# SergioRAgostinho/cvxpnpl

Measured on AMD Instinct MI355X. Metric: poses/sec (batched 10x10 SDP solves/sec), higher is better.
Workload: dtype f64

## Files before the change

### cvxpnpl_amd/csrc/cvxpnpl_hip.hip

```cpp
#include <hip/hip_runtime.h>
#include <stdint.h>
#include <stdio.h>
#include <string.h>
#include <unistd.h>

#include <map>
#include <memory>
#include <mutex>
#include <vector>
#include <utility>

#include "../../include/cvxpnpl_amd.h"
#include "problem_io.h"
#include "solver_core.h"
#include "lane_core.h"
#include "batch_args.h"
#include "wave_kernel.h"
#include "quad_kernel.h"
#include "ipm_quad.h"
#include "score_kernel.h"
#include "assemble_kernel.h"
#include "synth_kernel.h"
#include "recover_kernel.h"

// ... 162 lines not shown
}

void launch_wave(int64_t wgrid, hipStream_t s, const cvxw::WaveArgs &w, const cvx::Opts &o)
{
    if (o.variant == cvx::VAR_RC) hipLaunchKernelGGL(cvxw::solve_wave_kernel<cvx::VAR_RC>, dim3((unsigned)wgrid), dim3(64 * cvxw::WPB), 0, s, w, o);
    else hipLaunchKernelGGL(cvxw::solve_wave_kernel<cvx::VAR_FULL>, dim3((unsigned)wgrid), dim3(64 * cvxw::WPB), 0, s, w, o);
}

void launch_resume(int64_t rgrid, hipStream_t s, const cvxw::WaveArgs &w, const cvx::Opts &o, int32_t *count, int32_t *entries, const double *ws, bool full)
{
    cvxw::ResumeArgs ra;
    ra.a = w; ra.o = o; ra.count_p = count; ra.entries = entries; ra.ws = ws;
    ra.ws_stride = full ? cvxw::RS_FULL : cvxw::RS_LANE; ra.ws_full = full ? 1 : 0;
    ra.count2 = nullptr; ra.entries2 = nullptr; ra.grid1 = 0;
    if (o.variant == cvx::VAR_RC) hipLaunchKernelGGL(cvxw::resume_wave_kernel_rc, dim3((unsigned)rgrid), dim3(64), 0, s, ra);
    else hipLaunchKernelGGL(cvxw::resume_wave_kernel, dim3((unsigned)rgrid), dim3(64), 0, s, ra);
}

void launch_rescue(int64_t batch, hipStream_t s, const cvxw::WaveArgs &w, const cvx::Opts &o, int32_t *count = nullptr, int32_t *entries = nullptr,
                   const double *ws = nullptr)
{
    const int64_t rgrid = batch < cvxw::RESUME_GRID_MAX ? batch : cvxw::RESUME_GRID_MAX;
    cvxw::ResumeArgs ra;
    ra.a = w; ra.o = o; ra.count_p = w.rq_count; ra.entries = w.rq_entries; ra.ws = ws; ra.ws_stride = cvxw::RS_FULL; ra.ws_full = 1;
    ra.count2 = count; ra.entries2 = entries; ra.grid1 = (int)rgrid;
    if (o.variant == cvx::VAR_RC) hipLaunchKernelGGL(cvxw::rescue_wave_kernel_rc, dim3((unsigned)(count ? 2 * rgrid : rgrid)), dim3(64), 0, s, ra);
    else hipLaunchKernelGGL(cvxw::rescue_wave_kernel, dim3((unsigned)(count ? 2 * rgrid : rgrid)), dim3(64), 0, s, ra);
}

void launch_ipm(int64_t batch, hipStream_t s, const cvxw::WaveArgs &w, const cvx::Opts &o, int32_t *count, int32_t *entries)
{
    const int64_t groups = (batch + 3) / 4;
    const int64_t grid = groups < cvxi::IPMQ_GRID_MAX ? groups : cvxi::IPMQ_GRID_MAX;
    cvxi::IpmQuadArgs ia;
    ia.batch = batch; ia.rho = o.rho; ia.rho_tail = o.rho_tail; ia.tail_from = o.tail_from;
    ia.rq_count = w.rq_count; ia.rq_entries = w.rq_entries; ia.count = count; ia.entries = entries; ia.ws = w.rq_ws; ia.stride = w.rq_stride;
    ia.entries_cap = (int)(batch + cvxw::RESUME_GRID_MAX < 0x7fffffffLL ? batch + cvxw::RESUME_GRID_MAX : 0x7fffffffLL);
    ia.qs_in = nullptr; ia.z_out = nullptr; ia.s_out = nullptr; ia.gap_out = nullptr; ia.it_out = nullptr;
    if (o.variant == cvx::VAR_RC) hipLaunchKernelGGL(cvxi::ipm_quad_kernel<cvx::VAR_RC>, dim3((unsigned)grid), dim3(64), 0, s, ia);
    else hipLaunchKernelGGL(cvxi::ipm_quad_kernel<cvx::VAR_FULL>, dim3((unsigned)grid), dim3(64), 0, s, ia);
}

int set_err(const char *what, hipError_t e)
{
    snprintf(g_err, sizeof(g_err), "%s: %s", what, hipGetErrorString(e));
    return -2;
}

cvx::Opts to_core(const cvxpnpl_opts_t *opts)
{
    cvx::Opts o = cvx::default_opts();
    if (opts) {
        o.eps = opts->eps; o.max_iters = opts->max_iters; o.rho = opts->rho; o.alpha = opts->alpha;
        o.first_check = opts->first_check; o.check_every = opts->check_every; o.res_tol = opts->res_tol;
        o.jacobi_sweeps = opts->jacobi_sweeps; o.jacobi_tol = opts->jacobi_tol; o.warm_start = opts->warm_start; o.rho_tail = opts->rho_tail; o.tail_from = opts->tail_from;
        o.variant = opts->variant;
        o.adapt_every = opts->adapt_every; o.adapt_from = opts->adapt_from; o.adapt_mu = opts->adapt_mu; o.adapt_tau = opts->adapt_tau;
        o.stall_from = opts->stall_from; o.stall_lam = opts->stall_lam; o.stall_res = opts->stall_res; o.stall_drop = opts->stall_drop;
        o.rescue_from = opts->rescue_from;
        o.f32_sweeps_until = opts->f32_sweeps_until;
        o.sweep_schedule = opts->sweep_schedule != 0;
        o.dual_shift = opts->dual_shift < 0.0 ? (opts->variant == CVXPNPL_VARIANT_RC ? 0.006 : cvx::DUAL_SHIFT_DEFAULT) : opts->dual_shift;
        o.dual_refine = opts->dual_refine != 0;
    }
    if (o.f32_sweeps_until < 0) o.f32_sweeps_until = cvx::F32_SWEEPS_DEFAULT;
    return o;
}

}

namespace cvxd {
template <int W>
__global__ void __launch_bounds__(256) calibration_copy_kernel(const char *src, char *dst, int64_t nbytes)
{
    const int64_t n = nbytes / W;
    for (int64_t i = (int64_t)blockIdx.x * 256 + threadIdx.x; i < n; i += (int64_t)gridDim.x * 256) {
        if (W == 4) reinterpret_cast<uint32_t *>(dst)[i] = reinterpret_cast<const uint32_t *>(src)[i];
        if (W == 8) reinterpret_cast<double *>(dst)[i] = reinterpret_cast<const double *>(src)[i];
        if (W == 16) reinterpret_cast<double2 *>(dst)[i] = reinterpret_cast<const double2 *>(src)[i];
    }
}
}

extern "C" {

void cvxpnpl_default_opts(cvxpnpl_opts_t *opts)
{
    cvx::Opts o = cvx::default_opts();
    opts->eps = o.eps; opts->max_iters = o.max_iters; opts->rho = o.rho; opts->alpha = o.alpha;
    opts->first_check = 0 ; opts->check_every = o.check_every; opts->res_tol = o.res_tol;
    opts->jacobi_sweeps = o.jacobi_sweeps; opts->jacobi_tol = o.jacobi_tol; opts->warm_start = o.warm_start; opts->rho_tail = o.rho_tail; opts->tail_from = o.tail_from; opts->lane_iters = -1; opts->layout = CVXPNPL_LAYOUT_AUTO; opts->variant = CVXPNPL_VARIANT_FULL;
    opts->adapt_every = o.adapt_every; opts->adapt_from = o.adapt_from; opts->adapt_mu = o.adapt_mu; opts->adapt_tau = o.adapt_tau;
    opts->stall_from = o.stall_from; opts->stall_lam = o.stall_lam; opts->stall_res = o.stall_res; opts->stall_drop = o.stall_drop;
    opts->rescue_from = o.rescue_from;
    opts->f32_sweeps_until = -1;
    opts->sweep_schedule = 1;
    opts->dual_shift = -1.0;
    opts->dual_refine = -1;
    opts->struct_size = (uint32_t)sizeof(cvxpnpl_opts_t);
}

size_t cvxpnpl_opts_size(void) { return sizeof(cvxpnpl_opts_t); }

int cvxpnpl_last_layout(void) { return g_last_layout; }

static int check_args(int64_t batch, int32_t n_p, const double *p2, const double *p3, int32_t n_l, const double *l2,
                      const double *l3, const double *K)
{
    if (batch < 0 || n_p < 0 || n_l < 0 || (n_p == 0 && n_l == 0) || !K || (n_p > 0 && (!p2 || !p3)) || (n_l > 0 && (!l2 || !l3))) {
        snprintf(g_err, sizeof(g_err), "cvxpnpl: bad arguments (batch=%lld n_p=%d n_l=%d)", (long long)batch, n_p, n_l);
        return -1;
    }
    return 0;
}

static int launch_solve(const BatchArgs &a, const cvxpnpl_opts_t *opts, void *stream)
{
    const int64_t batch = a.batch;
    if (!a.R || !a.t || !a.status) { snprintf(g_err, sizeof(g_err), "cvxpnpl: R, t and status outputs are required"); return -1; }
    if (opts && opts->struct_size != (uint32_t)sizeof(cvxpnpl_opts_t)) {
        snprintf(g_err, sizeof(g_err), "cvxpnpl: options block of %u bytes, this library's cvxpnpl_opts_t has %zu (cvxpnpl_default_opts / cvxpnpl_opts_size)",
                 opts->struct_size, sizeof(cvxpnpl_opts_t));
        return -1;
    }
    if (opts && (opts->max_iters < 1 || opts->f32_sweeps_until < -1 || opts->f32_sweeps_until > cvx::F32_SWEEPS_DEFAULT || !(opts->rho > 0) || !(opts->eps > 0) || opts->check_every < 1 || opts->first_check < 0 ||
                 (opts->variant != CVXPNPL_VARIANT_FULL && opts->variant != CVXPNPL_VARIANT_RC) || opts->adapt_every < 0 ||
                 (opts->adapt_every > 0 && !(opts->adapt_mu >= 1.0 && opts->adapt_tau > 1.0)) || opts->rescue_from < -1 || !((opts->dual_shift >= 0.0 && opts->dual_shift <= 1.0) || opts->dual_shift == -1.0) || opts->dual_refine < -1 || opts->dual_refine > 1)) {
        snprintf(g_err, sizeof(g_err), "cvxpnpl: bad options");
        return -1;
    }
#ifdef CVXPNPL_EXPERIMENTS
    const bool layout_known = !opts || (opts->layout >= CVXPNPL_LAYOUT_AUTO && opts->layout <= CVXPNPL_LAYOUT_PENTA) || (opts->layout >= 9 && opts->layout <= 13);
#else
    const bool layout_known = !opts || (opts->layout >= CVXPNPL_LAYOUT_AUTO && opts->layout <= CVXPNPL_LAYOUT_PENTA);
#endif
    if (!layout_known) { snprintf(g_err, sizeof(g_err), "cvxpnpl: bad options (layout %d is not one of CVXPNPL_LAYOUT_*)", opts->layout); return -1; }
    cvx::Opts o = to_core(opts);
    if (!opts) o.first_check = 0;
    int cur_dev = 0;
    if (hipGetDevice(&cur_dev) != hipSuccess) { snprintf(g_err, sizeof(g_err), "cvxpnpl: hipGetDevice failed"); return -2; }
    std::lock_guard<std::mutex> launch_lock(launch_mutex(cur_dev, stream));
    hipStream_t s = (hipStream_t)stream;
    const int block = 64;
    int64_t grid = (batch + block - 1) / block;
    if (grid > 0x7fffffffLL) { snprintf(g_err, sizeof(g_err), "cvxpnpl: batch too large for one launch"); return -1; }
    int layout = opts ? opts->layout : CVXPNPL_LAYOUT_AUTO;
#ifdef CVXPNPL_EXPERIMENTS
    const bool layout_auto_like = layout == CVXPNPL_LAYOUT_AUTO || layout == 11 || layout == 12 || layout == 13;
#else
    const bool layout_auto_like = layout == CVXPNPL_LAYOUT_AUTO;
#endif
#ifdef CVXPNPL_EXPERIMENTS
    const bool minimal = !a.Q45 && a.n_p + a.n_l <= 4 && o.variant == cvx::VAR_FULL && layout_auto_like && batch >= 2560 && o.max_iters > 24;
#else
    const bool minimal = !a.Q45 && a.n_p + a.n_l <= 4 && o.variant == cvx::VAR_FULL && layout_auto_like && batch >= 2560 && o.max_iters > 24 &&
                         (!opts || opts->lane_iters <= 0);
#endif
    if (layout == CVXPNPL_LAYOUT_AUTO) layout = batch < 2560 ? CVXPNPL_LAYOUT_WAVE : ((batch < 20000 || minimal) ? CVXPNPL_LAYOUT_QUAD : CVXPNPL_LAYOUT_LANE);
    const bool rc = o.variant == cvx::VAR_RC;
    if (rc && (layout == CVXPNPL_LAYOUT_LANE || layout == CVXPNPL_LAYOUT_PENTA || layout == 9 || layout == 10 || layout == 12 || layout == 13)) layout = CVXPNPL_LAYOUT_QUAD;
    cvxw::WaveArgs w;
    w.batch = batch; w.n_p = a.n_p; w.n_l = a.n_l; w.K_per_problem = a.K_per_problem;
    w.p2 = a.p2; w.p3 = a.p3; w.l2 = a.l2; w.l3 = a.l3; w.K = a.K;
    w.R = a.R; w.t = a.t; w.cost = a.cost; w.Z = a.Z; w.status = a.status; w.iters = a.iters; w.work = a.work;
    w.Q45 = a.Q45; w.B27 = a.B27;
    w.rq_count = nullptr; w.rq_entries = nullptr;
    int quad_iters = opts ? opts->lane_iters : -1;
    if (quad_iters <= 0 && rc) quad_iters = 36;
    if (quad_iters <= 0 && minimal) quad_iters = 24;
    if (quad_iters <= 0) quad_iters = 7;
    if (quad_iters > 48) quad_iters = 48;
    if (quad_iters > 16 && !rc && !minimal) quad_iters = 16;
#ifdef CVXPNPL_EXPERIMENTS
    const bool lane_general = layout == 10;
    if (lane_general) layout = CVXPNPL_LAYOUT_LANE;
#else
    const bool lane_general = false;
#endif
    const bool penta_req = layout == CVXPNPL_LAYOUT_PENTA;
    const bool penta = penta_req && !(o.f32_sweeps_until < quad_iters);
    if (layout == 9 || layout == 11 || layout == 12 || layout == 13 || penta_req) layout = CVXPNPL_LAYOUT_QUAD;
    int lane_iters = opts ? opts->lane_iters : -1;
    {
        const int fc_lane = o.first_check > 0 ? o.first_check : 6;
        if (lane_iters <= 0) lane_iters = fc_lane;
        if (lane_iters > 6) lane_iters = 6;
#ifndef CVXPNPL_EXPERIMENTS
        const bool budgeted = !lane_general && fc_lane == lane_iters && lane_iters >= 2 && o.warm_start != 0;
        if (layout == CVXPNPL_LAYOUT_LANE && !budgeted) {
            layout = batch >= 2560 ? CVXPNPL_LAYOUT_QUAD : CVXPNPL_LAYOUT_WAVE;
            quad_iters = 7;
        }
#endif
    }
    if (layout == CVXPNPL_LAYOUT_QUAD && !(quad_iters >= 1 && o.max_iters > quad_iters)) layout = CVXPNPL_LAYOUT_WAVE;
    const bool minimal_queued = minimal && layout == CVXPNPL_LAYOUT_QUAD;
    const bool minimal_queued_f64 = minimal_queued && o.f32_sweeps_until < quad_iters;
    if (o.first_check <= 0) o.first_check = rc ? (layout == CVXPNPL_LAYOUT_QUAD ? 19 : 11) : (minimal_queued ? 17 : (minimal ? 7 : (layout == CVXPNPL_LAYOUT_LANE ? 6 : 5)));
    if (o.rescue_from < 0) {
        const int n = a.Q45 ? 8 : a.n_p + a.n_l;
        o.rescue_from = n <= 6 ? 32 : (n == 7 ? 64 : 128);
        if (rc) o.rescue_from = 48;
    }
    const bool rescue = o.rescue_from > 0 && o.max_iters > o.rescue_from;
    const bool lane_budgeted = !lane_general && o.first_check == lane_iters && lane_iters >= 2 && o.warm_start != 0;
    g_last_layout = (layout == CVXPNPL_LAYOUT_QUAD && penta) ? CVXPNPL_LAYOUT_PENTA : layout;
    const bool lane_hybrid = layout == CVXPNPL_LAYOUT_LANE && o.max_iters > lane_iters;
#ifndef CVXPNPL_FUSED_IPM
    const bool split = rescue && (rc || (!a.Q45 && a.n_p + a.n_l <= 5));
#else
    const bool split = false;
#endif
    WsView wv = {nullptr, nullptr, nullptr, nullptr, nullptr};
    const int ws_stride = layout == CVXPNPL_LAYOUT_QUAD ? cvxw::RS_FULL : ((lane_hybrid || split) ? cvxw::RS_LANE : 0);
    if (rescue || layout == CVXPNPL_LAYOUT_QUAD || lane_hybrid) {
        if (!get_workspace(batch, ws_stride, stream, wv)) return -2;
    }
    w.rq_ws = nullptr; w.rq_stride = 0;
    if (rescue) { w.rq_count = wv.rq_count; w.rq_entries = wv.rq_entries; }
    if (split) { w.rq_ws = wv.parked; w.rq_stride = ws_stride; }
    const int64_t rgrid_all = batch < cvxw::RESUME_GRID_MAX ? batch : cvxw::RESUME_GRID_MAX;
    if (layout == CVXPNPL_LAYOUT_QUAD) {
        int32_t *count = wv.count, *entries = wv.entries;
        double *ws = wv.parked;
        const int64_t qgrid = penta ? (batch + 4) / 5 : (batch + 3) / 4;
        cvxq::QuadArgs qa;
        qa.a = w; qa.o = o; qa.handoff_at = quad_iters; qa.qcount = count; qa.qentries = entries; qa.ws = ws;
#ifdef CVXPNPL_EXPERIMENTS
        if (opts && opts->layout == 9) hipLaunchKernelGGL((cvxq::solve_quad_kernel<1, 3>), dim3((unsigned)qgrid), dim3(64), 0, s, qa);
        else if (opts && opts->layout == 11 && rc) hipLaunchKernelGGL((cvxq::solve_quad_kernel<2, 3, 16, false, cvx::VAR_RC>), dim3((unsigned)qgrid), dim3(64), 0, s, qa);
        else if (opts && opts->layout == 11) hipLaunchKernelGGL((cvxq::solve_quad_kernel<2, 3>), dim3((unsigned)qgrid), dim3(64), 0, s, qa);
        else if (opts && opts->layout == 13) hipLaunchKernelGGL((cvxq::solve_quad_kernel<3, 2>), dim3((unsigned)qgrid), dim3(64), 0, s, qa);
        else if (opts && opts->layout == 12) hipLaunchKernelGGL((cvxq::solve_quad_kernel<2, 2>), dim3((unsigned)qgrid), dim3(64), 0, s, qa);
        else
#endif
        if (minimal_queued_f64) hipLaunchKernelGGL((cvxq::solve_quad_kernel<2, 2, 16, true>), dim3((unsigned)qgrid), dim3(64), 0, s, qa);
        else if (minimal_queued)
            hipLaunchKernelGGL((cvxq::solve_quad_kernel<2, 3>), dim3((unsigned)qgrid), dim3(64), 0, s, qa);
        else if (penta) hipLaunchKernelGGL((cvxq::solve_quad_kernel<0, 2, 12>), dim3((unsigned)qgrid), dim3(64), 0, s, qa);
        else if (rc && o.f32_sweeps_until < quad_iters) hipLaunchKernelGGL((cvxq::solve_quad_kernel<0, 2, 16, true, cvx::VAR_RC>), dim3((unsigned)qgrid), dim3(64), 0, s, qa);
        else if (rc) hipLaunchKernelGGL((cvxq::solve_quad_kernel<0, 2, 16, false, cvx::VAR_RC>), dim3((unsigned)qgrid), dim3(64), 0, s, qa);
        else if (o.f32_sweeps_until < quad_iters) hipLaunchKernelGGL((cvxq::solve_quad_kernel<0, 2, 16, true>), dim3((unsigned)qgrid), dim3(64), 0, s, qa);
        else hipLaunchKernelGGL((cvxq::solve_quad_kernel<0, 2>), dim3((unsigned)qgrid), dim3(64), 0, s, qa);
        const int64_t rgrid = batch < cvxw::RESUME_GRID_MAX ? batch : cvxw::RESUME_GRID_MAX;
        if (split) {
            for (int round = 0; round < 2; ++round) {
                launch_ipm(batch, s, w, o, count, entries);
                launch_resume(rgrid, s, w, o, count, entries, ws, true);
            }
        } else if (rescue) launch_rescue(batch, s, w, o, count, entries, ws);
        else launch_resume(rgrid, s, w, o, count, entries, ws, true);
    } else if (layout == CVXPNPL_LAYOUT_WAVE) {
        int64_t wgrid = (batch + cvxw::WPB - 1) / cvxw::WPB;
        if (wgrid > 0x7fffffffLL) { snprintf(g_err, sizeof(g_err), "cvxpnpl: batch too large for one launch"); return -1; }
        launch_wave(wgrid, s, w, o);
    } else {
        if (lane_hybrid) {
            int32_t *count = wv.count, *entries = wv.entries;
            double *ws = wv.parked;
            const bool budgeted = lane_budgeted;
            if (budgeted) cvxb::launch_lane2(!(o.f32_sweeps_until >= lane_iters), (unsigned)grid, (unsigned)block, (void *)s, a, o, lane_iters, count, entries, ws);
#ifdef CVXPNPL_EXPERIMENTS
            else if (o.f32_sweeps_until < lane_iters) hipLaunchKernelGGL(solve_lane_kernel<true>, dim3((unsigned)grid), dim3(block), 0, s, a, o, lane_iters, count, entries, ws);
            else hipLaunchKernelGGL(solve_lane_kernel<false>, dim3((unsigned)grid), dim3(block), 0, s, a, o, lane_iters, count, entries, ws);
#endif
            const int64_t rgrid = batch < cvxw::RESUME_GRID_MAX ? batch : cvxw::RESUME_GRID_MAX;
            launch_resume(rgrid, s, w, o, count, entries, ws, false);
        } else {
            int64_t wgrid = (batch + cvxw::WPB - 1) / cvxw::WPB;
            launch_wave(wgrid, s, w, o);
        }
    }
    if (split && layout != CVXPNPL_LAYOUT_QUAD) {
        launch_ipm(batch, s, w, o, wv.count, wv.entries);
        launch_resume(rgrid_all, s, w, o, wv.count, wv.entries, wv.parked, false);
    } else if (rescue && layout != CVXPNPL_LAYOUT_QUAD) launch_rescue(batch, s, w, o);
    hipError_t e = hipGetLastError();
    if (e != hipSuccess) return set_err("solve kernel launch", e);
    return 0;
}

int cvxpnpl_solve_batch(int64_t batch, int32_t n_p, const double *d_pts_2d, const double *d_pts_3d, int32_t n_l,
                        const double *d_line_2d, const double *d_line_3d, const double *d_K, int32_t K_per_problem,
                        const cvxpnpl_opts_t *opts, double *d_R, double *d_t, int32_t *d_status, int32_t *d_iters,
                        double *d_cost, double *d_Z, int32_t *d_work, void *stream)
{
    if (batch == 0) return 0;
    if (check_args(batch, n_p, d_pts_2d, d_pts_3d, n_l, d_line_2d, d_line_3d, d_K)) return -1;
    BatchArgs a;
    a.batch = batch; a.n_p = n_p; a.n_l = n_l; a.K_per_problem = K_per_problem;
    a.p2 = d_pts_2d; a.p3 = d_pts_3d; a.l2 = d_line_2d; a.l3 = d_line_3d; a.K = d_K;
    a.R = d_R; a.t = d_t; a.cost = d_cost; a.Z = d_Z; a.status = d_status; a.iters = d_iters; a.work = d_work;
    a.Q45 = nullptr; a.B27 = nullptr;
    return launch_solve(a, opts, stream);
}

int cvxpnpl_solve_cost_batch(int64_t batch, const double *d_Q45, const double *d_B27, const cvxpnpl_opts_t *opts, double *d_R,
                             double *d_t, int32_t *d_status, int32_t *d_iters, double *d_cost, double *d_Z, int32_t *d_work, void *stream)
{
    if (batch == 0) return 0;
    if (batch < 0 || !d_Q45 || !d_B27) { snprintf(g_err, sizeof(g_err), "cvxpnpl_solve_cost_batch: bad arguments (batch=%lld)", (long long)batch); return -1; }
    BatchArgs a;
    memset(&a, 0, sizeof(a));
    a.batch = batch;
    a.R = d_R; a.t = d_t; a.cost = d_cost; a.Z = d_Z; a.status = d_status; a.iters = d_iters; a.work = d_work;
    a.Q45 = d_Q45; a.B27 = d_B27;
    return launch_solve(a, opts, stream);
}

int cvxpnpl_assemble_batch(int64_t batch, int32_t n_p, const double *d_pts_2d, const double *d_pts_3d, int32_t n_l,
                           const double *d_line_2d, const double *d_line_3d, const double *d_K, int32_t K_per_problem,
                           double *d_B, double *d_Q45, void *stream)
{
    if (check_args(batch, n_p, d_pts_2d, d_pts_3d, n_l, d_line_2d, d_line_3d, d_K) || !d_B) return -1;
    if (batch == 0) return 0;
    BatchArgs a;
    memset(&a, 0, sizeof(a));
    a.batch = batch; a.n_p = n_p; a.n_l = n_l; a.K_per_problem = K_per_problem;
    a.p2 = d_pts_2d; a.p3 = d_pts_3d; a.l2 = d_line_2d; a.l3 = d_line_3d; a.K = d_K;
    const int block = 64;
    hipLaunchKernelGGL(assemble_kernel, dim3((unsigned)((batch + block - 1) / block)), dim3(block), 0, (hipStream_t)stream, a, d_B, d_Q45);
    hipError_t e = hipGetLastError();
    if (e != hipSuccess) return set_err("assemble_kernel launch", e);
    return 0;
}

// ... 372 lines not shown
```

### cvxpnpl_amd/csrc/quad_kernel.h

```cpp
#pragma once
#include <hip/hip_runtime.h>

#include "problem_io.h"
#include "solver_core.h"
#include "wave_kernel.h"

namespace cvxq {

using cvxw::WaveArgs;

constexpr int Q_WF = 0;
constexpr int Q_QF = 100;
constexpr int Q_Y = 200;
constexpr int Q_X = Q_Y + 40;
constexpr int Q_B = 324;
constexpr int Q_M = 352;
#ifndef CVXQ_SLICE
#define CVXQ_SLICE 388
#endif
constexpr int QLDS = CVXQ_SLICE;
constexpr int C_RED = 388;
constexpr int QLDS12 = 404;
template <int LPP> struct Geo {
    static constexpr int NPW = LPP == 16 ? 4 : 5;
// ... 285 lines not shown
#pragma unroll
    for (int i = 2; i < 10; i += 2) { s0 = fma(a[i], b[i], s0); s1 = fma(a[i + 1], b[i + 1], s1); }
    return s0 + s1;
}
__device__ __forceinline__ void jstep_dpp(double (&qd)[10], double &alq, bool real, bool tie_neg, bool active, double tol2, bool &coarse)
{
    double oq[10];
#pragma unroll
    for (int i = 0; i < 10; ++i) oq[i] = dpp_mov<0xB1>(qd[i]);
    const double be = dpp_mov<0xB1>(alq);
    const double gam = dot10_f64(qd, oq);
    const double g2 = gam * gam, ab = alq * be;
    coarse |= real && g2 > tol2 * ab;
    double c, sn, t;
    pair_cs_f64(be - alq, gam, active && real && g2 > 1e-30 * ab, tie_neg, c, sn, t);
#pragma unroll
    for (int i = 0; i < 10; ++i) qd[i] = c * qd[i] - sn * oq[i];
    alq += t;
}
__device__ __forceinline__ void jstep_bperm(double (&qd)[10], double &alq, int addr, bool real, bool tie_neg, bool take, bool active, double tol2, bool &coarse)
{
    double oq[10];
#pragma unroll
    for (int i = 0; i < 10; ++i) oq[i] = bperm(addr, qd[i]);
    const double be = bperm(addr, alq);
    const double gam = dot10_f64(qd, oq);
    const double g2 = gam * gam, ab = alq * be;
    coarse |= real && g2 > tol2 * ab;
    double c, sn, t;
    pair_cs_f64(be - alq, gam, active && real && g2 > 1e-30 * ab, tie_neg, c, sn, t);
    const double ka = take ? sn : c, kb = take ? c : -sn;
#pragma unroll
    for (int i = 0; i < 10; ++i) qd[i] = fma(ka, qd[i], kb * oq[i]);
    alq = take ? be - t : alq + t;
}
template <class COL, class T>
__device__ __forceinline__ void jacobi_sweep(COL &q, T &al, unsigned atab, int gl, int lane_base4, bool active, T tol2, bool &coarse)
{
    const bool col_lane = gl < 10;
#pragma unroll
    for (int st = 0; st < 9; ++st) {
        if ((st & 1) == 0) {
            jstep_dpp(q, al, col_lane, (gl & 1) != 0, active, tol2, coarse);
        } else {
            const int xs = st >> 1;
            const int partner = (int)((atab >> (4 * xs)) & 15u);
            jstep_bperm(q, al, lane_base4 + (partner << 2), partner != gl, gl > partner, ((atab >> (16 + xs)) & 1u) != 0, active, tol2, coarse);
        }
    }
}

template <class OWN>
__device__ __forceinline__ double quad_ldl(double *L, const OWN &w, double *Me)
{
    double minp = 1e300;
#pragma unroll
    for (int k = 0; k < 10; ++k) {
#pragma unroll
        for (int m = 0; m < OWN::EPL; ++m)
            if (w.ok(m) && w.ei(m) == k) L[C_ROW + w.ej(m)] = Me[m];
        CVXW_SYNC();
        const double d = L[C_ROW + k];
        minp = d < minp ? d : minp;
        const double id = cvxw::fast_rcp(d);
#pragma unroll
        for (int m = 0; m < OWN::EPL; ++m) {
            const double ra = L[C_ROW + w.ei(m)], rb = L[C_ROW + w.ej(m)];
            if (w.ei(m) > k) Me[m] -= ra * id * rb;
        }
        CVXW_SYNC();
    }
    return minp;
}


__device__ __forceinline__ void park(double *p, double x) { __hip_atomic_store(p, x, __ATOMIC_RELAXED, __HIP_MEMORY_SCOPE_AGENT); }

struct QuadArgs {
    WaveArgs a;
    cvx::Opts o;
    int handoff_at;
    int32_t *qcount, *qentries;
    double *ws;
};
typedef const __attribute__((address_space(4))) QuadArgs *QuadArgsPtr;

template <int NPW, int VAR>
__device__ __forceinline__ void finish_own(QuadArgsPtr kp, unsigned parked, double *lds)
{
#if defined(__HIP_DEVICE_COMPILE__)
    const WaveArgs a = kp->a;
    const cvx::Opts o = kp->o;
    const double *ws = kp->ws;
    const int64_t b0 = (int64_t)blockIdx.x * NPW;
    for (int g = 0; g < NPW; ++g) {
        if (!((parked >> g) & 1u)) continue;
        cvxw::solve_one_wave<VAR>(a, o, b0 + g, lds, ws + (b0 + g) * cvxw::RS_FULL, true);
        CVXW_SYNC();
    }
#endif
}

template <int MODE, int OCC = 2, int LPP = 16, bool F64SW = false, int VAR = cvx::VAR_FULL>
__global__ void __launch_bounds__(64, OCC) solve_quad_kernel(QuadArgs k)
{
    typedef Geo<LPP> G_;
    constexpr int NPW = G_::NPW, EPL = G_::EPL, SLICE = G_::SLICE;
    const WaveArgs &a = k.a;
    const cvx::Opts &o = k.o;
    const int handoff_at = k.handoff_at;
    int32_t *const qcount = k.qcount, *const qentries = k.qentries;
    double *const ws = k.ws;
    __shared__ __attribute__((aligned(16))) double lds_all[G_::NGRP * SLICE];
    const int lane = threadIdx.x & 63;
    const int grp = LPP == 16 ? lane >> 4 : (lane * 43) >> 9;
    const int gl = lane - grp * LPP;
    double *L = lds_all + grp * SLICE;
    double2 *L2 = reinterpret_cast<double2 *>(L);
    const int64_t b_raw = (int64_t)blockIdx.x * NPW + grp;
    const bool gvalid = grp < NPW && b_raw < a.batch;
    const int64_t b = gvalid ? b_raw : a.batch - 1;
#ifdef CVXQ_TIMELINE
    unsigned long long tl_[4];
    auto tl_now = []() { unsigned long long t; asm volatile("s_waitcnt vmcnt(0) lgkmcnt(0)\n\ts_memrealtime %0\n\ts_waitcnt lgkmcnt(0)" : "=s"(t) : : "memory"); return t; };
    tl_[0] = tl_now();
#endif

    Own<LPP> w;
    w.gl = gl;
#pragma unroll
    for (int m = 0; m < EPL; ++m) w.pk[m] = kETab.w[gl + LPP * m];
    const unsigned atab = kATab.w[gl];
    const int lane_base4 = (grp * LPP) << 2;

    bool okK = true, okG = true;
    double Qs[EPL];
    if (a.Q45) {
#pragma unroll
        for (int m = 0; m < EPL; ++m) Qs[m] = (w.ok(m) && w.ej(m) < 9) ? a.Q45[b * 45 + cvx::qidx(w.ei(m), w.ej(m))] : 0.0;
#pragma unroll
        for (int m = 0; m < G_::M27; ++m)
            if (gl + LPP * m < 27) L[Q_B + gl + LPP * m] = a.B27[b * 27 + gl + LPP * m];
    } else {
        cvx::ProblemView pv = cvx::make_view(b, a.n_p, a.p2, a.p3, a.n_l, a.l2, a.l3, a.K, a.K_per_problem);
        double Ki[9];
        {
            double Kc[9], det;
#pragma unroll
            for (int i = 0; i < 9; ++i) Kc[i] = pv.K[i];
            cvx::inv3(Kc, Ki, det);
            okK = (det == det) && det != 0.0;
        }
        constexpr int M60 = G_::M60;
        int rqa[M60], rqb[M60], rte[M60];
        double acc[M60];
#pragma unroll
        for (int m = 0; m < M60; ++m) acc[m] = 0.0;
#pragma unroll
        for (int m = 0; m < M60; ++m) {
            const int r = gl + LPP * m;
            const int al = r < 60 ? r : 0;
            int qa = 0, qb = 0, te = al;
            if (al >= 6 && al < 24) { qa = 1 + (al - 6) / 6; te = (al - 6) % 6; }
            if (al >= 24) {
                const int ab = (al - 24) / 6;
                te = (al - 24) % 6;
                qa = 1 + (ab < 3 ? 0 : (ab < 5 ? 1 : 2));
                qb = 1 + (ab < 3 ? ab : (ab < 5 ? ab - 2 : 2));
            }
            rqa[m] = 6 + qa; rqb[m] = 6 + qb; rte[m] = te;
        }
        const int nrec = pv.n_p + 2 * pv.n_l;
        double cs_[3];
        cvx::shift_centre(pv.n_p, pv.p3, pv.n_l, pv.l3, cs_);
        const double cs0 = cs_[0], cs1 = cs_[1], cs2 = cs_[2];
        for (int base = 0; base < nrec; base += LPP) {
            const int cnt = nrec - base < LPP ? nrec - base : LPP;
            if (gl < cnt) {
                const int r = base + gl;
                double T[6], P[3];
                if (r < pv.n_p) {
                    double p[3];
                    cvx::bearing(Ki, pv.p2[2 * r], pv.p2[2 * r + 1], p);
                    const double n2 = p[0] * p[0] + p[1] * p[1] + p[2] * p[2];
                    T[0] = n2 - p[0] * p[0]; T[1] = -p[0] * p[1]; T[2] = -p[0] * p[2];
                    T[3] = n2 - p[1] * p[1]; T[4] = -p[1] * p[2]; T[5] = n2 - p[2] * p[2];
                    P[0] = pv.p3[3 * r] - cs0; P[1] = pv.p3[3 * r + 1] - cs1; P[2] = pv.p3[3 * r + 2] - cs2;
                } else {
                    const int li = (r - pv.n_p) >> 1, en = (r - pv.n_p) & 1;
                    const double *l2 = pv.l2 + 4 * li, *l3 = pv.l3 + 6 * li + 3 * en;
                    double u[3], v[3];
                    cvx::bearing(Ki, l2[0], l2[1], u);
                    cvx::bearing(Ki, l2[2], l2[3], v);
                    double n[3] = {u[1] * v[2] - u[2] * v[1], u[2] * v[0] - u[0] * v[2], u[0] * v[1] - u[1] * v[0]};
                    const double inv = cvx::rsqrt_(n[0] * n[0] + n[1] * n[1] + n[2] * n[2]);
                    n[0] *= inv; n[1] *= inv; n[2] *= inv;
                    T[0] = n[0] * n[0]; T[1] = n[0] * n[1]; T[2] = n[0] * n[2]; T[3] = n[1] * n[1]; T[4] = n[1] * n[2]; T[5] = n[2] * n[2];
                    P[0] = l3[0] - cs0; P[1] = l3[1] - cs1; P[2] = l3[2] - cs2;
                }
                double *rec = L + Q_WF + gl * 10;
#pragma unroll
                for (int i = 0; i < 6; ++i) rec[i] = T[i];
                rec[6] = 1.0; rec[7] = P[0]; rec[8] = P[1]; rec[9] = P[2];
            }
            CVXW_SYNC();
            for (int c = 0; c < cnt; ++c) {
                const double *rec = L + Q_WF + c * 10;
#pragma unroll
// ... 451 lines not shown
                quad_proj<VAR>(L, w, T, 0.0);
#pragma unroll
                for (int m = 0; m < EPL; ++m) {
                    S[m] = odd[m] ? 0.0 : S[m] - T[m];
                    if (w.ok(m)) { L[Q_WF + w.ei(m) * 10 + w.ej(m)] = S[m]; L[Q_WF + w.ej(m) * 10 + w.ei(m)] = S[m]; }
                }
            }
            CVXW_SYNC();
            if (gl < 10) L[C_ROW + gl] = cvxw::dot10(L2 + (Q_WF + gl * 10) / 2, L2 + C_XV / 2);
            CVXW_SYNC();
            {
                double rhs[10], lamv[10];
#pragma unroll
                for (int i = 0; i < 10; ++i) rhs[i] = L[C_ROW + i];
                cvx::dual_lambda<VAR>(Rc, rhs, symm, lamv);
                if (gl == 0) {
#pragma unroll
                    for (int i = 0; i < 10; ++i) L[C_LAM + i] = lamv[i];
                }
            }
            CVXW_SYNC();
            {
                double E[EPL], Nn[EPL];
#pragma unroll
                for (int m = 0; m < EPL; ++m) {
                    E[m] = odd[m] ? 0.0 : 0.5 * (L[C_LAM + w.ei(m)] * L[C_XV + w.ej(m)] + L[C_XV + w.ei(m)] * L[C_LAM + w.ej(m)]);
                    Nn[m] = E[m];
                }
                quad_proj<VAR>(L, w, Nn, 0.0);
#pragma unroll
                for (int m = 0; m < EPL; ++m) {
                    S[m] -= E[m] - Nn[m];
                    if (w.ok(m)) { L[Q_WF + w.ei(m) * 10 + w.ej(m)] = S[m]; L[Q_WF + w.ej(m) * 10 + w.ei(m)] = S[m]; }
                }
            }
            CVXW_SYNC();
            double res, zSz;
            {
                const int aa = gl < 10 ? gl : 0;
                const double sz = cvxw::dot10(L2 + (Q_WF + aa * 10) / 2, L2 + C_XV / 2);
                res = grp_max<LPP>(L, gl, gl < 10 ? fabs(sz) : 0.0);
                zSz = grp_sum<LPP>(L, gl, gl < 10 ? L[C_XV + aa] * sz : 0.0);
            }
            CVXW_SYNC();
            double Se[EPL];
#pragma unroll
            for (int m = 0; m < EPL; ++m) Se[m] = S[m] + (((w.pk[m] >> 23) & 1) ? delta : 0.0);
CVXQ_PH(5);
            const double minp = quad_ldl(L, w, Se);
            const bool pre = (res < 1e-10) && (d0 > 0) && (pobj == pobj);
            const bool cok = (minp > 0) && pre;
            const bool gap_ok = cok && (tr * (fabs(zSz) + 4.0 * delta) <= gap_tol);
            have_prev = d0 > 0 && (pobj == pobj);
            fprev = pobj;
            if (gl == 0) {
#pragma unroll
                for (int i = 0; i < 9; ++i) { L[Q_M + 12 + i] = Rc[i]; L[Q_M + i] = Rc[i]; }
            }
            CVXW_SYNC();
            next_check = cvx::next_check_after(it, o);
            if (gap_ok && !done) {
                if (gl < 9) a.R[b * 9 + gl] = L[Q_M + gl];
                if (gl < 3) {
                    double tv = 0;
#pragma unroll
                    for (int c3 = 0; c3 < 3; ++c3)
#pragma unroll
                        for (int r3 = 0; r3 < 3; ++r3) tv += L[Q_B + gl * 9 + 3 * c3 + r3] * L[Q_M + r3 * 3 + c3];
                    a.t[b * 3 + gl] = -tv;
                }
                if (gl == 0) {
                    a.status[b] = cvx::ST_CERTIFIED;
                    if (a.iters) a.iters[b] = it;
                    if (a.cost) { a.cost[2 * b] = tr * pobj; a.cost[2 * b + 1] = tr * (pobj - zSz - 4.0 * delta); }
                    if (a.work) { a.work[2 * b] = 1; a.work[2 * b + 1] = total_sweeps; }
                }
                if (a.Z) {
#pragma unroll
                    for (int m = 0; m < EPL; ++m)
                        if (w.ok(m)) a.Z[b * 55 + w.e(m)] = L[C_XV + w.ei(m)] * L[C_XV + w.ej(m)];
                }
                done = true;
            }
        }
CVXQ_PH(6);
        if (!done && it == o.tail_from) {
#pragma unroll
            for (int m = 0; m < EPL; ++m) W[m] = Wp[m] + (W[m] - Wp[m]) * (rho / o.rho_tail);
        }
        if (it == o.tail_from) { rho = o.rho_tail; irho = 1.0 / rho; }
        {
            double X[EPL];
#pragma unroll
            for (int m = 0; m < EPL; ++m) X[m] = 2.0 * Wp[m] - W[m] - irho * (w.ej(m) < 9 ? L[Q_QF + w.ei(m) * 10 + w.ej(m)] : 0.0);
            quad_proj<VAR>(L, w, X, 1.0);
            double r2 = 0.0;
#pragma unroll
            for (int m = 0; m < EPL; ++m) {
                const double dd = X[m] - Wp[m];
                W[m] += o.alpha * dd;
                r2 += w.wgt(m) * dd * dd;
            }
            const double fp_res = cvx::sqrt_fast(grp_sum<LPP>(L, gl, r2));
            if (!done && !(fp_res == fp_res)) {
                if (gl < 9) a.R[b * 9 + gl] = NAN;
                if (gl < 3) a.t[b * 3 + gl] = NAN;
                if (gl == 0) {
                    a.status[b] = cvx::ST_NONFINITE;
                    if (a.iters) a.iters[b] = it;
                    if (a.cost) { a.cost[2 * b] = NAN; a.cost[2 * b + 1] = NAN; }
                    if (a.work) { a.work[2 * b] = 0; a.work[2 * b + 1] = total_sweeps; }
                }
                if (a.Z) {
#pragma unroll
                    for (int m = 0; m < EPL; ++m)
                        if (w.ok(m)) a.Z[b * 55 + w.e(m)] = NAN;
                }
                done = true;
            }
        }
CVXQ_PH(7);
        if (it >= handoff_at) {
            if (!done) {
                double *slot = ws + b * cvxw::RS_FULL;
#pragma unroll
                for (int m = 0; m < EPL; ++m)
                    if (w.ok(m)) {
                        park(slot + cvxw::RS_W + w.e(m), W[m]);
                        park(slot + cvxw::RS_Q + w.e(m), w.ej(m) < 9 ? L[Q_QF + w.ei(m) * 10 + w.ej(m)] * tr : 0.0);
                    }
#pragma unroll
                for (int m = 0; m < G_::M27; ++m)
                    if (gl + LPP * m < 27) park(slot + cvxw::RS_B + gl + LPP * m, L[Q_B + gl + LPP * m]);
                if (gl < 10) {
#pragma unroll
                    for (int i = 0; i < 10; ++i) park(slot + cvxw::RS_V + gl * 10 + i, vrow(i));
                }
                if (gl == 0) { park(slot + cvxw::RS_IT, (double)it); park(slot + cvxw::RS_NC, (double)next_check); }
                parked = true;
            }
            break;
        }
    }

#ifdef CVXQ_TIMELINE
    tl_[2] = tl_now();
#endif
    const unsigned long long pm = __ballot(parked);
    unsigned pmask = 0;
#pragma unroll
    for (int g = 0; g < NPW; ++g) pmask |= (unsigned)((pm >> (LPP * g)) & 1ull) << g;
    if (MODE == 1 || MODE == 2) {
        if (parked && gvalid && gl == 0) {
            const int q = atomicAdd(qcount, 1);
            qentries[q] = (int32_t)b;
        }
        return;
    }
    if (MODE == 3 && (pmask & (pmask - 1))) {
        const unsigned keep = pmask & (0u - pmask);
        const int g = grp < NPW ? grp : 0;
        if (parked && gvalid && gl == 0 && !((keep >> g) & 1u)) {
            const int q = atomicAdd(qcount, 1);
            qentries[q] = (int32_t)b;
        }
        pmask = keep;
// ... 30 lines not shown
```

Before: 56.41 million.

## Raise wave priority for second-round blocks and lagging solves in quad kernel

Queries occupancy once per device to find how many quad-kernel blocks fit in the first residency round. Blocks launched after that round raise their hardware wave priority with s_setprio. Waves that still hold unconverged problems at a convergence check raise their priority further. The aim is to shorten the tail where late or slow waves finish after the rest, at the cost of a host occupancy query, one extra kernel argument, and a scheduling effect that may not help.

```diff
diff --git a/cvxpnpl_amd/csrc/cvxpnpl_hip.hip b/cvxpnpl_amd/csrc/cvxpnpl_hip.hip
--- a/cvxpnpl_amd/csrc/cvxpnpl_hip.hip
+++ b/cvxpnpl_amd/csrc/cvxpnpl_hip.hip
@@ -268,6 +268,33 @@
 }
 }
 
+template <int MODE, int OCC, int LPP, bool F64SW, int VAR>
+static int quad_first_round(int dev)
+{
+#ifdef CVXQ_NO_PRIO
+    return 0;
+#else
+    static std::mutex mu;
+    static int slots[64] = {};
+    if (dev < 0 || dev >= 64) return 0;
+    std::lock_guard<std::mutex> g(mu);
+    if (!slots[dev]) {
+        int per_cu = 0, cus = 0;
+        const bool ok = hipOccupancyMaxActiveBlocksPerMultiprocessor(&per_cu, cvxq::solve_quad_kernel<MODE, OCC, LPP, F64SW, VAR>, 64, 0) == hipSuccess &&
+                        hipDeviceGetAttribute(&cus, hipDeviceAttributeMultiprocessorCount, dev) == hipSuccess && per_cu > 0 && cus > 0;
+        slots[dev] = ok ? per_cu * cus : -1;
+        if (!ok) (void)hipGetLastError();
+    }
+    return slots[dev];
+#endif
+}
+template <int MODE, int OCC = 2, int LPP = 16, bool F64SW = false, int VAR = cvx::VAR_FULL>
+static void launch_quad(int64_t qgrid, hipStream_t s, cvxq::QuadArgs &qa, int dev)
+{
+    qa.first_round = quad_first_round<MODE, OCC, LPP, F64SW, VAR>(dev);
+    hipLaunchKernelGGL((cvxq::solve_quad_kernel<MODE, OCC, LPP, F64SW, VAR>), dim3((unsigned)qgrid), dim3(64), 0, s, qa);
+}
+
 extern "C" {
 
 void cvxpnpl_default_opts(cvxpnpl_opts_t *opts)
@@ -411,23 +438,23 @@
         double *ws = wv.parked;
         const int64_t qgrid = penta ? (batch + 4) / 5 : (batch + 3) / 4;
         cvxq::QuadArgs qa;
-        qa.a = w; qa.o = o; qa.handoff_at = quad_iters; qa.qcount = count; qa.qentries = entries; qa.ws = ws;
+        qa.a = w; qa.o = o; qa.handoff_at = quad_iters; qa.qcount = count; qa.qentries = entries; qa.ws = ws; qa.first_round = 0;
 #ifdef CVXPNPL_EXPERIMENTS
-        if (opts && opts->layout == 9) hipLaunchKernelGGL((cvxq::solve_quad_kernel<1, 3>), dim3((unsigned)qgrid), dim3(64), 0, s, qa);
-        else if (opts && opts->layout == 11 && rc) hipLaunchKernelGGL((cvxq::solve_quad_kernel<2, 3, 16, false, cvx::VAR_RC>), dim3((unsigned)qgrid), dim3(64), 0, s, qa);
-        else if (opts && opts->layout == 11) hipLaunchKernelGGL((cvxq::solve_quad_kernel<2, 3>), dim3((unsigned)qgrid), dim3(64), 0, s, qa);
-        else if (opts && opts->layout == 13) hipLaunchKernelGGL((cvxq::solve_quad_kernel<3, 2>), dim3((unsigned)qgrid), dim3(64), 0, s, qa);
-        else if (opts && opts->layout == 12) hipLaunchKernelGGL((cvxq::solve_quad_kernel<2, 2>), dim3((unsigned)qgrid), dim3(64), 0, s, qa);
+        if (opts && opts->layout == 9) launch_quad<1, 3>(qgrid, s, qa, cur_dev);
+        else if (opts && opts->layout == 11 && rc) launch_quad<2, 3, 16, false, cvx::VAR_RC>(qgrid, s, qa, cur_dev);
+        else if (opts && opts->layout == 11) launch_quad<2, 3>(qgrid, s, qa, cur_dev);
+        else if (opts && opts->layout == 13) launch_quad<3, 2>(qgrid, s, qa, cur_dev);
+        else if (opts && opts->layout == 12) launch_quad<2, 2>(qgrid, s, qa, cur_dev);
         else
 #endif
-        if (minimal_queued_f64) hipLaunchKernelGGL((cvxq::solve_quad_kernel<2, 2, 16, true>), dim3((unsigned)qgrid), dim3(64), 0, s, qa);
+        if (minimal_queued_f64) launch_quad<2, 2, 16, true>(qgrid, s, qa, cur_dev);
         else if (minimal_queued)
-            hipLaunchKernelGGL((cvxq::solve_quad_kernel<2, 3>), dim3((unsigned)qgrid), dim3(64), 0, s, qa);
-        else if (penta) hipLaunchKernelGGL((cvxq::solve_quad_kernel<0, 2, 12>), dim3((unsigned)qgrid), dim3(64), 0, s, qa);
-        else if (rc && o.f32_sweeps_until < quad_iters) hipLaunchKernelGGL((cvxq::solve_quad_kernel<0, 2, 16, true, cvx::VAR_RC>), dim3((unsigned)qgrid), dim3(64), 0, s, qa);
-        else if (rc) hipLaunchKernelGGL((cvxq::solve_quad_kernel<0, 2, 16, false, cvx::VAR_RC>), dim3((unsigned)qgrid), dim3(64), 0, s, qa);
-        else if (o.f32_sweeps_until < quad_iters) hipLaunchKernelGGL((cvxq::solve_quad_kernel<0, 2, 16, true>), dim3((unsigned)qgrid), dim3(64), 0, s, qa);
-        else hipLaunchKernelGGL((cvxq::solve_quad_kernel<0, 2>), dim3((unsigned)qgrid), dim3(64), 0, s, qa);
+            launch_quad<2, 3>(qgrid, s, qa, cur_dev);
+        else if (penta) launch_quad<0, 2, 12>(qgrid, s, qa, cur_dev);
+        else if (rc && o.f32_sweeps_until < quad_iters) launch_quad<0, 2, 16, true, cvx::VAR_RC>(qgrid, s, qa, cur_dev);
+        else if (rc) launch_quad<0, 2, 16, false, cvx::VAR_RC>(qgrid, s, qa, cur_dev);
+        else if (o.f32_sweeps_until < quad_iters) launch_quad<0, 2, 16, true>(qgrid, s, qa, cur_dev);
+        else launch_quad<0, 2>(qgrid, s, qa, cur_dev);
         const int64_t rgrid = batch < cvxw::RESUME_GRID_MAX ? batch : cvxw::RESUME_GRID_MAX;
         if (split) {
             for (int round = 0; round < 2; ++round) {
diff --git a/cvxpnpl_amd/csrc/quad_kernel.h b/cvxpnpl_amd/csrc/quad_kernel.h
--- a/cvxpnpl_amd/csrc/quad_kernel.h
+++ b/cvxpnpl_amd/csrc/quad_kernel.h
@@ -391,7 +391,17 @@
     int handoff_at;
     int32_t *qcount, *qentries;
     double *ws;
+    int first_round;
 };
+
+#ifndef CVXQ_NO_PRIO
+#ifndef CVXQ_PRIO_ROUND2
+#define CVXQ_PRIO_ROUND2 1
+#endif
+#ifndef CVXQ_PRIO_BEHIND
+#define CVXQ_PRIO_BEHIND 2
+#endif
+#endif
 typedef const __attribute__((address_space(4))) QuadArgs *QuadArgsPtr;
 
 template <int NPW, int VAR>
@@ -433,6 +443,9 @@
     unsigned long long tl_[4];
     auto tl_now = []() { unsigned long long t; asm volatile("s_waitcnt vmcnt(0) lgkmcnt(0)\n\ts_memrealtime %0\n\ts_waitcnt lgkmcnt(0)" : "=s"(t) : : "memory"); return t; };
     tl_[0] = tl_now();
+#endif
+#if !defined(CVXQ_NO_PRIO) && CVXQ_PRIO_ROUND2 > 0
+    if (k.first_round > 0 && __builtin_amdgcn_readfirstlane((int)blockIdx.x) >= k.first_round) __builtin_amdgcn_s_setprio(CVXQ_PRIO_ROUND2);
 #endif
 
     Own<LPP> w;
@@ -1050,6 +1063,9 @@
                 }
                 done = true;
             }
+#if !defined(CVXQ_NO_PRIO) && CVXQ_PRIO_BEHIND > 0
+            if (__builtin_amdgcn_readfirstlane(__any(!done))) __builtin_amdgcn_s_setprio(CVXQ_PRIO_BEHIND);
+#endif
         }
 CVXQ_PH(6);
         if (!done && it == o.tail_from) {
```

Measured after the change: 57.96 million, median of 6. 1.03x the previous value.
